# reverb-sys/aeron-cluster-client-cpp

Measured on AMD Instinct MI355X. Metric: SBE records encoded+decoded/sec (device-resident), 256 B Order msgs, higher is better.
Workload: dtype u8; 1 GPU; roundtrip_fixed256_orders; records_per_gpu=1000000, record_bytes=256, encode=wire-correct TopicMessage, packed SoA input, decode=parse_message descriptors (views) + sequence_number evaluation, parallelism=shard1, input_sets=3

## Files before the change

### aeron-cluster-client-cpp_amd/csrc/sbe_codec.hip

```cpp
#include <hip/hip_ext.h>
#include <hip/hip_runtime.h>
#include <dlfcn.h>
#include <rccl/rccl.h>

#include <chrono>
#include <mutex>
#include <new>
#include <thread>
#include <type_traits>

#include <cstdint>
#include <cstdio>
#include <cstring>

#include "../../include/sbecodec.h"

namespace {

constexpr int kWave = 64;
constexpr int kTile = 64;
#ifndef SBE_DEC_WIN
#define SBE_DEC_WIN 16384
#endif
#ifndef SBE_DEC_WIN_WIDE
#define SBE_DEC_WIN_WIDE 20480
#endif
constexpr uint32_t kWin = SBE_DEC_WIN;
constexpr uint32_t kWinWide = SBE_DEC_WIN_WIDE;
constexpr uint64_t kWideAvg = 256;
#ifndef SBE_DEC_SMALL_AVG
#define SBE_DEC_SMALL_AVG 112
#endif
#ifndef SBE_DEC_MID_AVG
#define SBE_DEC_MID_AVG 204
#endif
#ifndef SBE_DEC_WIN_MID
#define SBE_DEC_WIN_MID 15360
#endif
constexpr uint32_t kWinMid = SBE_DEC_WIN_MID, kWinSmall = 8192;
#ifndef SBE_DEC_WIN_LARGE
#define SBE_DEC_WIN_LARGE 13312
#endif
#ifndef SBE_DEC_LARGE_AVG
#define SBE_DEC_LARGE_AVG 320
#endif
constexpr uint32_t kWinLarge = SBE_DEC_WIN_LARGE;
constexpr uint64_t kLargeAvg = SBE_DEC_LARGE_AVG;
constexpr uint64_t kMidAvg = SBE_DEC_MID_AVG, kSmallAvg = SBE_DEC_SMALL_AVG;

__device__ __forceinline__ uint32_t swz(uint32_t i) { return i ^ ((i >> 6) & 28u); }

__device__ __forceinline__ uint4 lds_read_chunk(const uint32_t* win, uint32_t c) {
    const uint32_t x = (c >> 4) & 31u;
    return *reinterpret_cast<const uint4*>(win + ((4u * c) ^ (x & 28u)));
}

__device__ __forceinline__ void lds_write_chunk(uint32_t* win, uint32_t c, uint4 v) {
    const uint32_t x = (c >> 4) & 31u;
    *reinterpret_cast<uint4*>(win + ((4u * c) ^ (x & 28u))) = v;
}

__device__ __forceinline__ uint32_t lds_dw(const uint32_t* win, uint32_t i) { return win[swz(i)]; }
__device__ __forceinline__ uint4 lds_read_chunk_raw(const uint32_t* win, uint32_t c) {
    return *reinterpret_cast<const uint4*>(win + ((4u * c) ^ (((c >> 4) & 31u) & 28u)));
}

template <int kCtrl, int kRowMask = 0xf>
__device__ __forceinline__ uint32_t dpp0(uint32_t v) {
    return (uint32_t)__builtin_amdgcn_update_dpp(0, (int)v, kCtrl, kRowMask, 0xf, false);
}

__device__ __forceinline__ uint32_t wave_incl_scan(uint32_t v, int lane) {
    (void)lane;
    v += dpp0<0x111>(v);
    v += dpp0<0x112>(v);
    v += dpp0<0x114>(v);
    v += dpp0<0x118>(v);
    v += dpp0<0x142, 0xa>(v);
    v += dpp0<0x143, 0xc>(v);
    return v;
}

__device__ __forceinline__ uint32_t ceil_div_small(uint32_t a, uint32_t b) {
    const uint32_t x = a + b - 1;
    uint32_t q = (uint32_t)((float)x * __builtin_amdgcn_rcpf((float)b));
    q += (q + 1) * b <= x;
    q -= q * b > x;
    return q;
}

__device__ __forceinline__ uint32_t wave_incl_max(uint32_t v) {
    v = max(v, dpp0<0x111>(v));
    v = max(v, dpp0<0x112>(v));
    v = max(v, dpp0<0x114>(v));
    v = max(v, dpp0<0x118>(v));
    v = max(v, dpp0<0x142, 0xa>(v));
    v = max(v, dpp0<0x143, 0xc>(v));
    return v;
}

template <int kCtrl, int kRowMask = 0xf>
__device__ __forceinline__ uint64_t dpp_add64(uint64_t v) {
    const uint32_t lo = (uint32_t)v, hi = (uint32_t)(v >> 32);
    const uint32_t tlo = dpp0<kCtrl, kRowMask>(lo), thi = dpp0<kCtrl, kRowMask>(hi);
    const uint32_t nlo = lo + tlo;
    return ((uint64_t)(hi + thi + (nlo < lo ? 1u : 0u)) << 32) | nlo;
}
__device__ __forceinline__ uint64_t wave_incl_scan64(uint64_t v, int lane) {
    (void)lane;
    v = dpp_add64<0x111>(v);
    v = dpp_add64<0x112>(v);
    v = dpp_add64<0x114>(v);
    v = dpp_add64<0x118>(v);
    v = dpp_add64<0x142, 0xa>(v);
    v = dpp_add64<0x143, 0xc>(v);
    return v;
}

__device__ __forceinline__ uint32_t lane_u32(uint32_t v, int l) { return __builtin_amdgcn_readlane(v, l); }
__device__ __forceinline__ uint64_t lane_u64(uint64_t v, int l) {
    const uint32_t hi = (uint32_t)__builtin_amdgcn_readlane((uint32_t)(v >> 32), l);
    const uint32_t lo = (uint32_t)__builtin_amdgcn_readlane((uint32_t)v, l);
    return ((uint64_t)hi << 32) | lo;
}

__device__ __forceinline__ uint64_t wave_sum64(uint64_t v) { return lane_u64(wave_incl_scan64(v, 0), kWave - 1); }

__device__ __forceinline__ uint64_t uniform64(uint64_t v) {
    uint32_t lo = __builtin_amdgcn_readfirstlane((uint32_t)v);
    uint32_t hi = __builtin_amdgcn_readfirstlane((uint32_t)(v >> 32));
    return ((uint64_t)hi << 32) | lo;
}

__device__ __forceinline__ uint32_t byte_mask_bits(uint32_t nbytes) {
    return nbytes >= 4 ? 0xffffffffu : ((1u << (8u * nbytes)) - 1u);
}

typedef unsigned int u32x4 __attribute__((ext_vector_type(4)));
typedef __attribute__((address_space(1))) const uint32_t g_u32;
typedef __attribute__((address_space(1))) const u32x4 g_u32x4;
__device__ __forceinline__ uint32_t gload32(uintptr_t addr) { return *reinterpret_cast<g_u32*>(addr); }
__device__ __forceinline__ uint4 gload128(uintptr_t addr) {
    const u32x4 v = *reinterpret_cast<g_u32x4*>(addr);
    return make_uint4(v.x, v.y, v.z, v.w);
}
__device__ __forceinline__ uint4 gload128_nt(uintptr_t addr) {
    const u32x4 v = __builtin_nontemporal_load(reinterpret_cast<g_u32x4*>(addr));
    return make_uint4(v.x, v.y, v.z, v.w);
}
template <typename T>
__device__ __forceinline__ void dst_store(T* p, T v) {
    __builtin_nontemporal_store(v, p);
}

constexpr int kSbThreads = 1024;
constexpr int kTilesPerSb = 2 * kWave;
constexpr int kSbRecMin = kTilesPerSb * 32;

template <int kPre_, int kBlk_, int kNF_, bool kTM_, int kRpt_>
struct Lay {
    static constexpr int kRpt = kRpt_;
    static constexpr int kLpr = kWave / kRpt;
    static constexpr int kSbRec = kTilesPerSb * kRpt;
    static_assert((kRpt == 32 || kRpt == 64) && kSbRec % kSbThreads == 0 && kSbThreads % kRpt == 0, "tile shape");
    static constexpr int32_t kPre = kPre_;
    static constexpr int32_t kBlk = kBlk_;
    static constexpr int kNF = kNF_;
    static constexpr bool kTM = kTM_;
    static constexpr int32_t kLit = kPre + 8 + kBlk;
    static constexpr int32_t kS0 = kLit + 2;
    static constexpr int32_t kOvh = kLit + 2 * kNF;
    static constexpr int32_t ovh(bool trunc) { return kOvh - (trunc ? 8 : 0); }
    static constexpr int kStoreRows0 = kNF == 2 ? (kRpt == 64 ? 5 : 3) : 8;
};
#ifndef SBE_TM_RPT
#define SBE_TM_RPT 32
#endif
#ifndef SBE_TMS_RPT
#define SBE_TMS_RPT 32
#endif
#ifndef SBE_L3_RPT
#define SBE_L3_RPT 64
#endif
using LayTM = Lay<0, 16, 5, true, SBE_TM_RPT>;
using LayTMS = Lay<32, 16, 5, true, SBE_TMS_RPT>;
using LayL2 = Lay<0, 12, 2, false, 64>;
using LayL3 = Lay<0, 12, 3, false, SBE_L3_RPT>;
static_assert(LayTM::kOvh == SBE_TM_WIRE_OVERHEAD && LayTM::ovh(true) == SBE_TM_REF_OVERHEAD, "TM layout");
static_assert(LayL2::kOvh == SBE_LITE_OVERHEAD(2) && LayTMS::kPre == SBE_SESSION_HDR_LEN, "layouts");
#define SBE_TILE_SHAPE(LY)                                                  \
    [[maybe_unused]] constexpr int kRpt = LY::kRpt, kLpr = LY::kLpr; \
    [[maybe_unused]] constexpr int kSbRec = LY::kSbRec

struct EncArgs {
    const uint8_t* arena;
    const uint32_t* str_off;
    const uint32_t* str_len;
    const uint64_t* timestamp;
    const uint32_t* topic_id;
    uint32_t tmpl;
    int64_t term_id, sess_id;
    uint64_t n;
    uint64_t ts_default;
    uint8_t* out;
    uint64_t cap;
    uint64_t* out_off;
    uint8_t* status;
    uint64_t* tsum;
    uint64_t* bsum;
    uint8_t* sink;
};
constexpr int kSinkBytes = 16 * 64;

constexpr int kOutAux = 2;
constexpr int kOutAuxKeep = 0;
constexpr uint64_t kKeepMin = 96ull << 20, kKeepMax = 256ull << 20;

enum : int { kLenWire = 0, kLenRef = 1, kLenPub = 2 };

template <class LY, int kLen>
__device__ __forceinline__ void rec_sizes(const EncArgs& a, uint64_t r, uint32_t& out_b, uint64_t& in_b,
                                          uint8_t& st) {
    uint32_t sum = 0;
    uint64_t sum_in = 0;
    st = SBE_ENC_OK;
    if (r < a.n) {
#pragma unroll
        for (int f = LY::kNF - 1; f >= 0; --f) {
            const uint32_t L = a.str_len[LY::kNF * r + f];
            sum += kLen == kLenPub ? (L & 0xffffu) : L;
            sum_in += L;
            if (kLen != kLenPub && L > SBE_VAR_MAX_LEN) st = (uint8_t)(SBE_ENC_E109_TOPIC + f);
        }
    }
    const uint32_t ovh = (uint32_t)LY::ovh(kLen == kLenRef);
    out_b = (r < a.n && st == SBE_ENC_OK) ? ovh + sum : 0u;
    in_b = r < a.n ? sum_in : 0u;
}


template <class LY, bool kPacked, int kLen>
__global__ __launch_bounds__(kSbThreads) void sbe_enc_sums(EncArgs a) {
    SBE_TILE_SHAPE(LY);
    __shared__ uint64_t tl[2][kTilesPerSb];
    const int tid = threadIdx.x;
    const uint64_t sb = blockIdx.x;
#pragma unroll
    for (int j = 0; j < kSbRec / kSbThreads; ++j) {
        const uint64_t r = sb * kSbRec + (uint64_t)j * kSbThreads + tid;
        uint32_t ob;
        uint64_t ib;
        uint8_t st;
        rec_sizes<LY, kLen>(a, r, ob, ib, st);
        const int lane = tid & (kWave - 1);
        const uint32_t so = wave_incl_scan(ob, lane);
        const uint32_t o31 = lane_u32(so, 31), o63 = lane_u32(so, kWave - 1);
        uint64_t i31 = 0, i63 = 0;
        if (kPacked) {
            const uint64_t si = wave_incl_scan64(ib, lane);
            i31 = lane_u64(si, 31);
            i63 = lane_u64(si, kWave - 1);
        }
        if (lane == 0) {
            const int tile = j * (kSbThreads / kRpt) + (kWave / kRpt) * (tid / kWave);
            if (kRpt == 32) {
                tl[0][tile] = o31;
                tl[1][tile] = i31;
                tl[0][tile + 1] = o63 - o31;
                tl[1][tile + 1] = i63 - i31;
            } else {
                tl[0][tile] = o63;
                tl[1][tile] = i63;
            }
        }
    }
    __syncthreads();
    if (tid < kWave) {
        const int lane = tid;
        constexpr int kPer = kTilesPerSb / kWave;
        const uint64_t o0 = tl[0][kPer * lane], o1 = kPer == 2 ? tl[0][kPer * lane + 1] : 0ull;
        const uint64_t i0 = tl[1][kPer * lane], i1 = kPer == 2 ? tl[1][kPer * lane + 1] : 0ull;
        const uint64_t io = wave_incl_scan64(o0 + o1, lane), ii = wave_incl_scan64(i0 + i1, lane);
        const uint64_t eo = io - o0 - o1, ei = ii - i0 - i1;
        const uint64_t t0 = sb * kTilesPerSb + kPer * lane;
        *reinterpret_cast<ulonglong2*>(a.tsum + 2 * t0) = make_ulonglong2(eo, ei);
        if (kPer == 2) *reinterpret_cast<ulonglong2*>(a.tsum + 2 * t0 + 2) = make_ulonglong2(eo + o0, ei + i0);
        if (lane == kWave - 1) *reinterpret_cast<ulonglong2*>(a.bsum + 2 * sb) = make_ulonglong2(io, ii);
    }
}

#ifndef SBE_PACK_MIN_WAVES
#define SBE_PACK_MIN_WAVES 1
#endif
#ifndef SBE_ENC_WIN
#define SBE_ENC_WIN 8192
#endif
constexpr int32_t kEW = SBE_ENC_WIN;
constexpr int32_t kEWIn = SBE_ENC_WIN + 256;

constexpr int32_t kInSlack = 64;
constexpr int32_t kRowPad = 16;
constexpr int32_t kWoutBytes = kEW + (kEW / 256) * kRowPad;
constexpr int32_t kWinBytes = kEWIn + 2 * kInSlack;

typedef __attribute__((address_space(3))) uint8_t lds_u8;
typedef __attribute__((address_space(3))) const uint8_t lds_cu8;
typedef __attribute__((address_space(3))) uint32_t lds_u32;
typedef __attribute__((address_space(3))) const uint32_t lds_cu32;
typedef unsigned int u32x2 __attribute__((ext_vector_type(2)));
typedef __attribute__((address_space(3))) u32x4 lds_u32x4;
typedef __attribute__((address_space(3))) u32x2 lds_u32x2;
__device__ __forceinline__ void lds_store16(lds_u8* p, uint4 v) {
    u32x4 x;
    x.x = v.x; x.y = v.y; x.z = v.z; x.w = v.w;
    *reinterpret_cast<lds_u32x4*>(p) = x;
}

__device__ __forceinline__ uint32_t wout_addr(int32_t d) { return (uint32_t)d + (((uint32_t)d >> 8) * kRowPad); }

struct LdsLin {
    lds_cu8* b;
    __device__ __forceinline__ uint32_t dw(int32_t i) const { return reinterpret_cast<lds_cu32*>(b)[i]; }
};
struct GlbClamp {
    uintptr_t base4;
    int32_t imax;
    __device__ __forceinline__ uint32_t dw(int32_t i) const {
        i = i < 0 ? 0 : (i > imax ? imax : i);
        return gload32(base4 + 4u * (uint32_t)i);
    }
};

__device__ __forceinline__ uint64_t low_bytes64(uint64_t v, int32_t n) { return n >= 8 ? v : v & ((1ull << (8 * n)) - 1); }

struct Writer {
    lds_u8* w;
    int32_t lo, pos;
    uint32_t carry;

    __device__ __forceinline__ void put_dw(int32_t d, uint32_t v) const {
        *reinterpret_cast<lds_u32*>(w + wout_addr(d)) = v;
    }
    __device__ __forceinline__ void put_bytes(int32_t d, uint32_t v, int32_t b0, int32_t b1) const {
        lds_u8* p = w + wout_addr(d);
#pragma unroll
        for (int k = 0; k < 4; ++k)
            if (k >= b0 && k < b1) p[k] = (uint8_t)(v >> (8 * k));
    }
    __device__ __forceinline__ void put_first(int32_t d, uint32_t v) const {
        if (d >= lo) put_dw(d, v); else put_bytes(d, v, lo - d, 4);
    }
    __device__ __forceinline__ void lit(uint64_t v, int32_t n) {
        const int32_t t = pos & 3, d = pos & ~3, total = t + n;
        const uint64_t lo64 = (v << (8 * t)) | carry;
        const uint32_t x0 = (uint32_t)lo64, x1 = (uint32_t)(lo64 >> 32);
        const uint32_t x2 = t ? (uint32_t)(v >> (64 - 8 * t)) : 0u;
        if (total >= 4) put_first(d, x0);
        if (total >= 8) put_dw(d + 4, x1);
        carry = total >= 8 ? x2 : (total >= 4 ? x1 : x0);
        pos += n;
    }
    template <typename Src>
    __device__ __forceinline__ void str(const Src& S, int32_t s, int32_t m) {
        const int32_t t = pos & 3, d = pos & ~3, total = t + m;
        const int32_t u = s - t;
        const uint32_t sh = (uint32_t)u & 3u;
        const int32_t i0 = u >> 2;
        const int32_t nd = total >> 2, rem = total & 3;
        uint32_t prev = S.dw(i0);
        const uint32_t nx = S.dw(i0 + 1);
        const uint32_t w0 = (__builtin_amdgcn_alignbyte(nx, prev, sh) & ~byte_mask_bits((uint32_t)t)) | carry;
        pos += m;
        if (nd == 0) {
            carry = w0 & byte_mask_bits((uint32_t)total);
            return;
        }
        put_first(d, w0);
        prev = nx;
        int32_t k = 1;
        const int32_t kg = 4 - ((d >> 2) & 3);
        for (; k < kg && k < nd; ++k) {
            const uint32_t n0 = S.dw(i0 + k + 1);
            put_dw(d + 4 * k, __builtin_amdgcn_alignbyte(n0, prev, sh));
            prev = n0;
        }
        for (; k + 4 <= nd; k += 4) {
            const uint32_t n0 = S.dw(i0 + k + 1), n1 = S.dw(i0 + k + 2), n2 = S.dw(i0 + k + 3), n3 = S.dw(i0 + k + 4);
            u32x2 lo2, hi2;
            lo2.x = __builtin_amdgcn_alignbyte(n0, prev, sh);
            lo2.y = __builtin_amdgcn_alignbyte(n1, n0, sh);
            hi2.x = __builtin_amdgcn_alignbyte(n2, n1, sh);
            hi2.y = __builtin_amdgcn_alignbyte(n3, n2, sh);
            lds_u8* g = w + wout_addr(d + 4 * k);
            reinterpret_cast<lds_u32x2*>(g)[0] = lo2;
            reinterpret_cast<lds_u32x2*>(g)[1] = hi2;
            prev = n3;
        }
        for (; k < nd; ++k) {
            const uint32_t n0 = S.dw(i0 + k + 1);
            put_dw(d + 4 * k, __builtin_amdgcn_alignbyte(n0, prev, sh));
            prev = n0;
        }
        carry = rem ? (__builtin_amdgcn_alignbyte(S.dw(i0 + nd + 1), prev, sh) & byte_mask_bits((uint32_t)rem)) : 0u;
    }
    __device__ __forceinline__ void flush() const {
        const int32_t t = pos & 3;
        if (t) {
            const int32_t d = pos & ~3;
            put_bytes(d, carry, lo > d ? lo - d : 0, t);
        }
    }
};

__device__ __noinline__ Writer str_global(Writer W, uintptr_t sa, int32_t m) {
    const uintptr_t b4 = sa & ~(uintptr_t)3;
    const int32_t sl = (int32_t)(sa - b4);
    W.str(GlbClamp{b4, (sl + m - 1) >> 2}, sl, m);
    return W;
}

__device__ __forceinline__ void wsync() { __builtin_amdgcn_wave_barrier(); }

constexpr int kStageRegs = (kEWIn / 16 + kWave - 1) / kWave;

#ifdef SBE_PACK_PHASES
__device__ uint64_t g_pack_phase[16384 * 8];
struct Ph {
    uint64_t t, acc[8];
    __device__ void start() {
        t = __builtin_amdgcn_s_memtime();
        for (int k = 0; k < 8; ++k) acc[k] = 0;
    }
    __device__ void lap(int k) {
        const uint64_t n = __builtin_amdgcn_s_memtime();
        acc[k] += n - t;
        t = n;
    }
    __device__ void put(int lane) {
        uint64_t v = 0;
        for (int k = 0; k < 8; ++k) v = lane == k ? acc[k] : v;
        if (lane < 8 && blockIdx.x < 16384) g_pack_phase[8 * blockIdx.x + lane] = v;
    }
};
#else
struct Ph {
    __device__ void start() {}
    __device__ void lap(int) {}
    __device__ void put(int) {}
};
#endif

struct TileIn {
    uint32_t L[5];
    uint64_t ts;
    uint32_t tid;
    uint64_t to, ti, po, pi;
    uint32_t pcount;
};

struct TileSt {
    uint32_t rs, rec_out, ps, pe;
    uint32_t pe_rec;
    uint64_t in0;
    uint32_t L[5];
    uint64_t ts;
    uint32_t tid;
    uint64_t T0;
    uint32_t len;
    uint32_t agg_in;
    uintptr_t in_tile;
    uintptr_t gsrc[5];
    bool wrapped;
    uint32_t agg_out;
    uint64_t tot_in;
};

template <class LY, bool kPacked>
__device__ __forceinline__ TileIn tile_load(const EncArgs& a, uint64_t tile, int lane, uint64_t& sb_next) {
    SBE_TILE_SHAPE(LY);
    TileIn x;
    uint64_t r = tile * kRpt + lane / kLpr;
    r = r < a.n ? r : a.n - 1;
#pragma unroll
    for (int f = 0; f < 5; ++f) x.L[f] = f < LY::kNF ? a.str_len[LY::kNF * r + f] : 0u;
    x.ts = a.timestamp[r];
    x.tid = LY::kTM ? 0u : a.topic_id[r];
    x.to = a.tsum[2 * tile];
    x.ti = kPacked ? a.tsum[2 * tile + 1] : 0ull;
    const uint64_t sbt = tile / kTilesPerSb;
    const uint64_t last_sb = (a.n - 1) / kSbRec;
    uint64_t s = sb_next + (uint64_t)lane;
    s = s < last_sb ? s : last_sb;
    x.po = a.bsum[2 * s];
    x.pi = kPacked ? a.bsum[2 * s + 1] : 0ull;
    x.pcount = sbt > sb_next ? (uint32_t)(sbt - sb_next) : 0u;
    sb_next = sbt > sb_next ? sbt : sb_next;
    return x;
}

template <class LY, bool kPacked, int kLen>
__device__ __forceinline__ TileSt tile_prepare_at(const EncArgs& a, const TileIn& x, uint64_t r_first, uint64_t rend,
                                                  int lane, uint64_t base_out, uint64_t base_in);

template <class LY, bool kPacked, int kLen>
__device__ __forceinline__ TileSt tile_prepare(const EncArgs& a, const TileIn& x, uint64_t tile, int lane,
                                               uint64_t& sp_out, uint64_t& sp_in) {
    SBE_TILE_SHAPE(LY);
    sp_out += wave_sum64((uint32_t)lane < x.pcount ? x.po : 0ull);
    if (kPacked) sp_in += wave_sum64((uint32_t)lane < x.pcount ? x.pi : 0ull);
    const uint64_t base_out = uniform64(sp_out + x.to);
    const uint64_t base_in = kPacked ? uniform64(sp_in + x.ti) : 0ull;
    return tile_prepare_at<LY, kPacked, kLen>(a, x, tile * kRpt, a.n, lane, base_out, base_in);
}

template <class LY, bool kPacked, int kLen>
__device__ __forceinline__ TileSt tile_prepare_at(const EncArgs& a, const TileIn& x, uint64_t r_first, uint64_t rend,
                                                  int lane, uint64_t base_out, uint64_t base_in) {
    SBE_TILE_SHAPE(LY);
    TileSt S;
    const int q = lane % kLpr;
    const uint64_t r = r_first + lane / kLpr;
    const bool valid = r < rend;
    uint64_t sum = 0, sum_in = 0;
    uint8_t st = SBE_ENC_OK;
#pragma unroll
    for (int f = 0; f < 5; ++f) {
        const uint32_t Lx = valid ? x.L[f] : 0u;
        S.L[f] = kLen == kLenPub ? (Lx & 0xffffu) : Lx;
        sum += S.L[f];
        sum_in += Lx;
    }
    if (kLen != kLenPub) {
#pragma unroll
        for (int f = LY::kNF - 1; f >= 0; --f)
            if (S.L[f] > SBE_VAR_MAX_LEN) st = (uint8_t)(SBE_ENC_E109_TOPIC + f);
    }
    const uint32_t ovh = (uint32_t)LY::ovh(kLen == kLenRef);
    const uint32_t rec_out = (valid && st == SBE_ENC_OK) ? ovh + (uint32_t)sum : 0u;
    const uint64_t rec_in = (kPacked && valid) ? sum_in : 0ull;
    S.wrapped = kLen == kLenPub && kPacked && __ballot(sum_in != sum) != 0;
    const uint32_t lo_out = q == 0 ? rec_out : 0u;
    const uint32_t inc_out = wave_incl_scan(lo_out, lane);
    const uint32_t agg_out = lane_u32(inc_out, kWave - 1);
    S.rs = kLpr == 2 ? dpp0<0xa0>(inc_out - lo_out) : inc_out - lo_out;
    S.rec_out = rec_out;
    S.agg_out = agg_out;
    S.tot_in = 0;
    if (kPacked) {
        if (__ballot(!(valid && st == SBE_ENC_OK)) == 0 && !S.wrapped) {
            const uint32_t ovh0 = ovh;
            S.in0 = S.rs - ovh0 * (uint32_t)(lane / kLpr);
            const uint64_t agg_in = agg_out - (uint64_t)ovh0 * kRpt;
            S.agg_in = (uint32_t)agg_in;
            S.tot_in = agg_in;
        } else {
            const uint64_t lo_in = q == 0 ? rec_in : 0ull;
            const uint64_t inc_in = wave_incl_scan64(lo_in, lane);
            const uint64_t agg_in = lane_u64(inc_in, kWave - 1);
            S.agg_in = agg_in < 0x7fffffffull ? (uint32_t)agg_in : 0x7fffffffu;
            S.tot_in = agg_in;
            const uint64_t ex = inc_in - lo_in;
            S.in0 = kLpr == 2 ? ((uint64_t)dpp0<0xa0>((uint32_t)(ex >> 32)) << 32) | dpp0<0xa0>((uint32_t)ex) : ex;
        }
    } else {
        S.agg_in = 0;
        S.in0 = 0;
    }
    S.ts = LY::kTM ? ((valid && x.ts) ? x.ts : a.ts_default) : x.ts;
    S.tid = x.tid;
    const uint32_t re = S.rs + rec_out;
    const uint64_t cap_rel64 = a.cap > base_out ? a.cap - base_out : 0ull;
    uint32_t cap_rel = agg_out;
    if (cap_rel64 < (uint64_t)agg_out) {
        const uint64_t over = __ballot(q == 0 && rec_out != 0 && (uint64_t)re > cap_rel64);
        cap_rel = lane_u32(S.rs, __builtin_ctzll(over));
    }
    if (valid && q == 0) {
        if (st == SBE_ENC_OK && (uint64_t)re > cap_rel64) st = SBE_ENC_OVERFLOW;
        a.out_off[r] = base_out + S.rs;
        if (r == a.n - 1) a.out_off[a.n] = base_out + re;
        if (a.status) a.status[r] = st;
    }
    const uint32_t ps = q == 0 ? S.rs : ((S.rs + (uint32_t)q * rec_out / kLpr + 3) & ~3u);
    const uint32_t pe = q == kLpr - 1 ? re : ((S.rs + (uint32_t)(q + 1) * rec_out / kLpr + 3) & ~3u);
    const uint32_t hi_rec = re < cap_rel ? re : cap_rel;
// ... 1737 lines not shown
        }
    }
    if (d.len[0] == 0) {
#pragma unroll
        for (int k = 0; k < 5; ++k) d.off[k] = d.len[k] = 0;
        d.status = SBE_ST_EG_NONE;
        return;
    }
    d.status = SBE_ST_EG_TM;
}

template <typename R_t>
__device__ void dec_lite(const R_t& R, uint32_t len, Desc& d) {
    d.clear();
    if (len < 8) { d.status = SBE_ST_LITE_NOT_LITE; return; }
    const uint32_t h0 = R.u32(0), h1 = R.u32(4);
    const uint32_t blk = h0 & 0xffffu, tmpl = h0 >> 16, schema = h1 & 0xffffu;
    d.set_hdr(R, 0);
    const uint32_t nf = tmpl == SBE_COMMIT_OFFSET_LITE_TEMPLATE_ID ? 2u
                      : (tmpl == SBE_ORDER_REQUEST_LITE_TEMPLATE_ID || tmpl == SBE_ORDER_NOTIFICATION_LITE_TEMPLATE_ID) ? 3u
                                                                                                                   : 0u;
    if (schema != 1 || nf == 0) { d.status = SBE_ST_LITE_NOT_LITE; return; }
    uint32_t pos = 8u + blk;
    if (pos > len || len < 20) { d.status = SBE_ST_LITE_E100; return; }
#pragma unroll
    for (uint32_t f = 0; f < 3; ++f) {
        if (f >= nf) break;
        if (pos + 2 > len) {
#pragma unroll
            for (int k = 0; k < 5; ++k) d.off[k] = d.len[k] = 0;
            d.status = SBE_ST_LITE_E100;
            return;
        }
        const uint32_t L = R.u16(pos);
        pos += 2;
        if (pos + L > len) {
#pragma unroll
            for (int k = 0; k < 5; ++k) d.off[k] = d.len[k] = 0;
            d.status = SBE_ST_LITE_E100;
            return;
        }
        d.off[f] = pos;
        d.len[f] = L;
        pos += L;
    }
    d.status = SBE_ST_LITE;
    d.ts = R.u64(12);
    d.off[4] = R.u32(8);
}

template <uint32_t kW>
constexpr int dec_regs() {
    static_assert(kW % (16 * kWave) == 0, "decode windows are whole 1 KiB staging rows");
    return (int)(kW / 16 / kWave);
}


template <uint32_t kMode, typename R_t>
__device__ __forceinline__ void dec_record(const R_t& R, uint32_t len, Desc& d) {
    if (kMode == SBE_DEC_ON_EGRESS)
        dec_on_egress(R, len, d);
    else if (kMode == SBE_DEC_LITE)
        dec_lite(R, len, d);
    else
        dec_parse_message(R, len, d);
}

template <uint32_t kMode>
__device__ __noinline__ Desc dec_record_glb(const uint8_t* in, uint64_t rs, uint32_t rl) {
    Desc d;
    d.clear();
    dec_record<kMode>(GlbRec{reinterpret_cast<uintptr_t>(in) + rs}, rl, d);
    return d;
}

template <uint32_t kW>
__device__ __forceinline__ void dec_issue(const DecArgs& a, uint64_t wb, uint64_t we, int lane,
                                          uint4 (&I)[dec_regs<kW>()]) {
    const uint32_t nch = (uint32_t)((we - wb) >> 4);
    const uintptr_t src = reinterpret_cast<uintptr_t>(a.in) + wb;
#pragma unroll
    for (int k = 0; k < dec_regs<kW>(); ++k) {
        const uint32_t ch = lane + kWave * k;
        I[k] = ch < nch ? gload128_nt(src + 16ull * ch) : make_uint4(0, 0, 0, 0);
    }
}

template <uint32_t kMode, uint32_t kW>
__device__ __forceinline__ uint32_t dec_commit(uint32_t* win, uint64_t wb, uint64_t we, bool wide, int lane,
                                               const uint4 (&I)[dec_regs<kW>()]) {
    const uint32_t nch = (uint32_t)((we - wb) >> 4);
#pragma unroll
    for (int k = 0; k < dec_regs<kW>(); ++k) {
        const uint32_t ch = lane + kWave * k;
        if (ch < nch) lds_write_chunk(win, ch, I[k]);
    }
    uint32_t sm = 0;
    if (kMode == SBE_DEC_PARSE_MESSAGE && wide) {
        const uint32_t nrow = (nch + kWave - 1) / kWave;
#pragma unroll
        for (int k = 0; k < dec_regs<kW>(); ++k) {
            if ((uint32_t)k < nrow) {
                Suspect S;
                S.add(I[k]);
                sm |= S.any() ? 1u << k : 0u;
            }
        }
    }
    return sm;
}

template <uint32_t kMode, uint32_t kW>
__device__ __forceinline__ uint32_t dec_stage(const DecArgs& a, uint32_t* win, uint64_t wb, uint64_t we, bool wide,
                                              int lane) {
    uint4 I[dec_regs<kW>()];
    dec_issue<kW>(a, wb, we, lane, I);
    return dec_commit<kMode, kW>(win, wb, we, wide, lane, I);
}

template <uint32_t kMode>
__device__ __forceinline__ void dec_window(const uint32_t* win, uint64_t wb, uint64_t we, uint64_t rs, uint64_t rl,
                                           bool wide, uint32_t sm, bool& done, Desc& d, int lane) {
    bool here = false;
    if (!done && rs >= wb && rs + rl <= we) {
        dec_record<kMode>(LdsRec{win, (uint32_t)(rs - wb)}, (uint32_t)rl, d);
        done = true;
        here = true;
    }
    if (kMode == SBE_DEC_PARSE_MESSAGE) {
        const bool pend = here && (d.flags & kFlSeqPending);
        if (!wide) {
            if (pend)
                d.flags = (d.flags & ~kFlSeqPending) | has_seq_key_lane(LdsRec{win, (uint32_t)(rs - wb)}, d.off[3], d.len[3]);
        } else if (__ballot(pend)) {
            uint32_t hit = 0;
            if (__ballot(sm != 0)) {
                uint32_t hpos;
                bool more;
                window_exact(win, sm, (uint32_t)(we - wb), lane, hpos, more);
                const uint32_t p0 = (uint32_t)(rs - wb) + d.off[3], p1 = p0 + d.len[3];
                if (__ballot(more)) {
                    if (pend) hit = has_seq_key_lane(LdsRec{win, (uint32_t)(rs - wb)}, d.off[3], d.len[3]);
                } else {
                    for (uint64_t m = __ballot(hpos != ~0u); m; m &= m - 1) {
                        const uint32_t x = __builtin_amdgcn_readlane(hpos, __builtin_ctzll(m));
                        const uint32_t xa = x & ~kHitEsc;
                        if (x & kHitEsc) hit |= xa >= p0 && xa < p1 ? SBE_FL_SEQ_ESC : 0u;
                        else hit |= x >= p0 && x + 16 <= p1 ? SBE_FL_SEQ_KEY : 0u;
                    }
                }
            }
            if (pend) d.flags = (d.flags & ~kFlSeqPending) | hit;
        }
    }
}

#ifndef SBE_DEC_MINW
#define SBE_DEC_MINW 3
#endif
#ifdef SBE_SERVE_PROF
__device__ uint64_t g_serve_prof[16];
#define SBE_SVP(k, t) tpk[(k) - 5] = __builtin_amdgcn_s_memrealtime()
#else
#define SBE_SVP(k, t) do { } while (0)
#endif
template <uint32_t kMode, uint32_t kWin>
__device__ __forceinline__ void dec_rest(const DecArgs& a, uint32_t* win, uint64_t T0, uint64_t end, uint64_t rs,
                                         uint64_t rl, bool wide, bool& done, Desc& d, int lane,
                                         uint4 (&I)[dec_regs<kWin>()]) {
    for (;;) {
        bool again = false;
        uint64_t wb = 0;
        for (;;) {
            const uint64_t m = __ballot(!done);
            if (m == 0) break;
            const int f = __builtin_ctzll(m);
            const uint64_t rsf = uniform64(__shfl(rs, f, kWave));
            const uint64_t rlf = uniform64(__shfl(rl, f, kWave));
            if ((rsf & 15) + rlf <= kWin && rsf + rlf <= end && rsf >= (T0 & ~15ull)) {
                wb = rsf & ~15ull;
                again = true;
                break;
            }
            if (lane == f) {
                d = dec_record_glb<kMode>(a.in, rs, (uint32_t)rl);
                done = true;
            }
        }
        if (!again) break;
        const uint64_t we = wb + kWin < end ? wb + kWin : end;
        wsync();
        dec_issue<kWin>(a, wb, we, lane, I);
        const uint32_t sm = dec_commit<kMode, kWin>(win, wb, we, wide, lane, I);
        wsync();
        dec_window<kMode>(win, wb, we, rs, rl, wide, sm, done, d, lane);
    }
}

template <uint32_t kMode, bool kServe>
__device__ __forceinline__ void dec_outputs(const DecArgs& a, uint64_t r, bool valid, uint64_t rs, const Desc& d) {
    if (valid) {
        dst_store(a.status + r, (uint8_t)d.status);
        dst_store(a.flags + r, (uint8_t)d.flags);
        dst_store(reinterpret_cast<uint64_t*>(a.hdr + 4 * r),
                  (uint64_t)((uint32_t)d.hdr[0] | ((uint32_t)d.hdr[1] << 16)) |
                      ((uint64_t)((uint32_t)d.hdr[2] | ((uint32_t)d.hdr[3] << 16)) << 32));
        dst_store(a.ts + r, d.ts);
    }
    if (valid) {
        typedef uint32_t u32x4a4 __attribute__((ext_vector_type(4), aligned(4)));
        u32x4a4 o4, l4;
        o4.x = d.off[0]; o4.y = d.off[1]; o4.z = d.off[2]; o4.w = d.off[3];
        l4.x = d.len[0]; l4.y = d.len[1]; l4.z = d.len[2]; l4.w = d.len[3];
        __builtin_nontemporal_store(o4, reinterpret_cast<u32x4a4*>(a.view_off + 5 * r));
        __builtin_nontemporal_store(d.off[4], a.view_off + 5 * r + 4);
        __builtin_nontemporal_store(l4, reinterpret_cast<u32x4a4*>(a.view_len + 5 * r));
        __builtin_nontemporal_store(d.len[4], a.view_len + 5 * r + 4);
    }
    if (kMode == SBE_DEC_PARSE_MESSAGE && a.seq) {
        const bool cand = valid && d.status == SBE_ST_TM && (d.flags & kSeqCand);
        if (__ballot(cand) && cand)
            a.seq[r] = kServe ? json_seq_eval_call_serve(a.in + rs + d.off[3], d.len[3])
                              : json_seq_eval_call(a.in + rs + d.off[3], d.len[3]);
    }
}

template <uint32_t kMode>
__device__ __forceinline__ void dec_oversize(Desc& d) {
    d.status = kMode == SBE_DEC_ON_EGRESS ? SBE_ST_EG_NONE
             : kMode == SBE_DEC_LITE    ? SBE_ST_LITE_E100
                                        : SBE_ST_ERR_TM_E100;
}

template <uint32_t kMode, uint32_t kWin, bool kServe = false>
__device__ __forceinline__ void dec_tile(const DecArgs& a, uint64_t tile, uint32_t* win) {
#ifdef SBE_SERVE_PROF
    const uint64_t tp0 = __builtin_amdgcn_s_memrealtime();
    uint64_t tpk[4] = {tp0, tp0, tp0, tp0};
#endif
    const int lane = threadIdx.x & (kWave - 1);
    const uint64_t t0 = tile * kTile;
    const uint64_t r = t0 + (uint64_t)lane;
    const bool valid = r < a.n;
    const uint64_t last = t0 + kTile < a.n ? t0 + kTile : a.n;
    const uint64_t T0 = uniform64(a.rec_off[t0]);
    const uint64_t end = (uniform64(a.rec_off[last]) + 15) & ~15ull;
    const uint64_t rc = r < a.n ? r : a.n - 1;
    const uint64_t rs = a.rec_off[rc];
    const uint64_t rl = valid ? a.rec_off[rc + 1] - rs : 0;

    Desc d;
    d.clear();
    bool done = !valid;
    if (valid && rl > 0xffffffffull) {
        dec_oversize<kMode>(d);
        done = true;
    }
    uint64_t wb = T0 & ~15ull;
    uint64_t we = wb + kWin < end ? wb + kWin : (end > wb ? end : wb);
    const bool wide = kServe || __ballot(valid && rl > kSeqLaneRec) != 0;
    uint4 I[dec_regs<kWin>()];
    SBE_SVP(5, tp0);
    dec_issue<kWin>(a, wb, we, lane, I);
    uint32_t sm = dec_commit<kMode, kWin>(win, wb, we, wide, lane, I);
    SBE_SVP(6, tp0);
    bool pre = false;
    uint64_t wb2 = 0, we2 = 0;
    {
        const uint64_t m = __ballot(!(done || (rs >= wb && rs + rl <= we)));
        if (m) {
            const int f = __builtin_ctzll(m);
            const uint64_t rsf = uniform64(__shfl(rs, f, kWave));
            const uint64_t rlf = uniform64(__shfl(rl, f, kWave));
            if ((rsf & 15) + rlf <= kWin && rsf + rlf <= end && rsf >= (T0 & ~15ull)) {
                wb2 = rsf & ~15ull;
                we2 = wb2 + kWin < end ? wb2 + kWin : end;
                pre = true;
                dec_issue<kWin>(a, wb2, we2, lane, I);
            }
        }
    }
    wsync();
    dec_window<kMode>(win, wb, we, rs, rl, wide, sm, done, d, lane);
    if (pre) {
        wsync();
        sm = dec_commit<kMode, kWin>(win, wb2, we2, wide, lane, I);
        wsync();
        dec_window<kMode>(win, wb2, we2, rs, rl, wide, sm, done, d, lane);
    }
    if (__ballot(!done)) dec_rest<kMode, kWin>(a, win, T0, end, rs, rl, wide, done, d, lane, I);
    SBE_SVP(7, tp0);
    dec_outputs<kMode, kServe>(a, r, valid, rs, d);
    SBE_SVP(8, tp0);
#ifdef SBE_SERVE_PROF
    if (kServe && lane == 0)
        for (int k = 0; k < 4; ++k) g_serve_prof[5 + k] += tpk[k] - tp0;
#endif
}

#ifndef SBE_DEC_MINW_WIDE
#define SBE_DEC_MINW_WIDE SBE_DEC_MINW
#endif
template <uint32_t kMode, uint32_t kWin>
__global__ __launch_bounds__(kWave, kWin == kWinWide && kWinWide > 16384 ? 2 : ((kWin == kWinWide || kWin == kWinLarge) ? SBE_DEC_MINW_WIDE : SBE_DEC_MINW)) void sbe_decode_kernel(DecArgs a) {
    __shared__ uint32_t win[kWin / 4];
    dec_tile<kMode, kWin>(a, blockIdx.x, win);
}

__device__ __forceinline__ uint64_t counted_n(const uint64_t* n_dev, uint64_t capacity) {
    const uint64_t c = uniform64(*n_dev);
    return c < capacity ? c : capacity;
}

template <uint32_t kMode, uint32_t kWin>
__global__ __launch_bounds__(kWave, kWin == kWinWide && kWinWide > 16384 ? 2 : ((kWin == kWinWide || kWin == kWinLarge) ? SBE_DEC_MINW_WIDE : SBE_DEC_MINW)) void sbe_decode_counted_kernel(DecArgs a, const uint64_t* n_dev) {
    __shared__ uint32_t win[kWin / 4];
    a.n = counted_n(n_dev, a.n);
    if ((uint64_t)blockIdx.x * kTile >= a.n) return;
    dec_tile<kMode, kWin>(a, blockIdx.x, win);
}

thread_local char g_last_error[256] = "";

int record_hip(hipError_t e) {
    if (e == hipSuccess) return SBE_OK;
    std::strncpy(g_last_error, hipGetErrorString(e), sizeof(g_last_error) - 1);
    return SBE_EHIP;
}

constexpr uint64_t kMaxTiles = 0xffffffffull;

uint64_t pack_grid(const void* kernel, uint64_t tiles) {
    struct Entry {
        const void* k;
        int dev;
        uint64_t g;
    };
    static thread_local Entry cache[32] = {};
    int dev = 0;
    if (hipGetDevice(&dev) != hipSuccess) dev = 0;
    uint64_t g = 0;
    for (const Entry& e : cache)
        if (e.k == kernel && e.dev == dev) g = e.g;
    if (g == 0) {
        int per_cu = 0, cus = 0;
        if (hipOccupancyMaxActiveBlocksPerMultiprocessor(&per_cu, kernel, kWave, 0) != hipSuccess || per_cu < 1)
            per_cu = 1;
        if (hipDeviceGetAttribute(&cus, hipDeviceAttributeMultiprocessorCount, dev) != hipSuccess || cus < 1)
            cus = 256;
        g = (uint64_t)per_cu * (uint64_t)cus;
        for (Entry& e : cache)
            if (e.k == nullptr) {
                e = Entry{kernel, dev, g};
                break;
            }
    }
    if (g > (uint64_t)(kWave - 1) * kTilesPerSb) g = (uint64_t)(kWave - 1) * kTilesPerSb;
    return tiles < g ? tiles : g;
}

struct ProfRing {
    static constexpr int kCap = 256;
    hipEvent_t ev[kCap][2];
    int head = 0, count = 0;
    uint64_t launches = 0;
    bool ready = false;
};
thread_local int g_prof_every = 0;
thread_local ProfRing g_prof[2];

hipError_t prof_ready(ProfRing& R) {
    if (!R.ready) {
        for (int i = 0; i < ProfRing::kCap; ++i)
            for (int j = 0; j < 2; ++j) {
                const hipError_t e = hipEventCreate(&R.ev[i][j]);
                if (e != hipSuccess) return e;
            }
        R.ready = true;
    }
    return hipSuccess;
}

void prof_slot(int which, hipEvent_t* start, hipEvent_t* stop) {
    *start = *stop = nullptr;
    if (g_prof_every <= 0) return;
    ProfRing& R = g_prof[which];
    if (R.launches++ % (uint64_t)g_prof_every != 0) return;
    if (!R.ready) return;
    *start = R.ev[R.head][0];
    *stop = R.ev[R.head][1];
}
void prof_commit(int which, hipEvent_t start) {
    if (!start) return;
    ProfRing& R = g_prof[which];
    R.head = (R.head + 1) % ProfRing::kCap;
    if (R.count < ProfRing::kCap) ++R.count;
}


struct FragScan {
    uint32_t dp;
    uint32_t sg;
    int32_t lb;
    int32_t le;
    uint64_t B, E;
};
constexpr uint32_t kFsCount = 0x7fffffffu;
__host__ __device__ __forceinline__ uint32_t fs_dp(const FragScan& e) { return e.dp & kFsCount; }
__host__ __device__ __forceinline__ uint32_t fs_sg(const FragScan& e) { return e.sg & kFsCount; }
struct FragScanOp {
    __host__ __device__ FragScan operator()(const FragScan& a, const FragScan& b) const {
        const bool Aa = (a.sg >> 31) != 0, Ab = (b.sg >> 31) != 0, Ca = (a.dp >> 31) != 0, Cb = (b.dp >> 31) != 0;
        const uint32_t C = (Ca || (Cb && Aa)) ? 0x80000000u : 0u, A = (Aa && Ab) ? 0x80000000u : 0u;
        return FragScan{((fs_dp(a) + fs_dp(b)) & kFsCount) | C, ((fs_sg(a) + fs_sg(b)) & kFsCount) | A,
                        a.lb > b.lb ? a.lb : b.lb, a.le > b.le ? a.le : b.le,
                        (Ab ? a.B : 0ull) + b.B, a.E + (Cb ? a.B : 0ull) + b.E};
    }
};

struct FragArgs {
    const uint8_t* in;
    const uint64_t* frag_off;
    const uint8_t* flags;
    uint64_t n;
    uint8_t* out;
    uint64_t* msg_off;
    uint64_t* counts;
    FragScan* el;
    FragScan* sc;
    uint64_t* msize;
    uint64_t* mfirst;
    uint64_t* mlast;
    uint64_t* big;
};
constexpr uint64_t kFcBig = 64 * 1024, kFcPiece = 64 * 1024;

__device__ __forceinline__ bool frag_single(uint8_t f) {
    return (f & (SBE_FRAG_BEGIN | SBE_FRAG_END)) == (SBE_FRAG_BEGIN | SBE_FRAG_END);
}

#ifndef SBE_FS_PER
#define SBE_FS_PER 4
#endif
constexpr int kFsPer = SBE_FS_PER, kFsThreads = 256, kFsBlk = kFsPer * kFsThreads;
__device__ __forceinline__ FragScan fs_identity() { return FragScan{0u, 0x80000000u, -1, -1, 0ull, 0ull}; }
__device__ __forceinline__ FragScan fs_elem(const FragArgs& a, uint64_t i) {
    if (i >= a.n) return fs_identity();
    const uint8_t f = a.flags[i];
    const bool single = frag_single(f);
    const bool begin = (f & SBE_FRAG_BEGIN) != 0, endf = (f & SBE_FRAG_END) != 0;
    const uint64_t len = a.frag_off[i + 1] - a.frag_off[i];
    FragScan e;
    e.dp = ((single || endf) ? 1u : 0u) | ((!single && endf) ? 0x80000000u : 0u);
    e.sg = (single ? 1u : 0u) | ((single || (!begin && !endf)) ? 0x80000000u : 0u);
    e.lb = (!single && begin) ? (int32_t)i : -1;
    e.le = (!single && endf) ? (int32_t)i : -1;
    e.B = (!single && !endf) ? len : 0ull;
    e.E = (single || endf) ? len : 0ull;
    return e;
}
__device__ __forceinline__ FragScan fs_shfl_up(const FragScan& v, int d) {
    FragScan t;
    t.dp = __shfl_up(v.dp, d, kWave);
    t.sg = __shfl_up(v.sg, d, kWave);
    t.lb = __shfl_up(v.lb, d, kWave);
    t.le = __shfl_up(v.le, d, kWave);
    t.B = __shfl_up(v.B, d, kWave);
    t.E = __shfl_up(v.E, d, kWave);
    return t;
}
__device__ __forceinline__ FragScan fs_wave_scan(FragScan v, int lane) {
#pragma unroll
    for (int d = 1; d < kWave; d <<= 1) {
        const FragScan t = fs_shfl_up(v, d);
        if (lane >= d) v = FragScanOp{}(t, v);
    }
    return v;
}
__device__ __forceinline__ FragScan fs_block(const FragArgs& a, uint64_t b, FragScan (&e)[kFsPer], FragScan* wt,
                                             FragScan& before) {
    const int tid = threadIdx.x, lane = tid & (kWave - 1), w = tid / kWave;
    const uint64_t i0 = b * kFsBlk + (uint64_t)tid * kFsPer;
#pragma unroll
    for (int k = 0; k < kFsPer; ++k) e[k] = fs_elem(a, i0 + k);
#pragma unroll
    for (int k = 1; k < kFsPer; ++k) e[k] = FragScanOp{}(e[k - 1], e[k]);
    const FragScan inc = fs_wave_scan(e[kFsPer - 1], lane);
    const FragScan up = fs_shfl_up(inc, 1);
    const FragScan ex = lane ? up : fs_identity();
    if (lane == kWave - 1) wt[w] = inc;
    __syncthreads();
    FragScan wpre = fs_identity(), tot = fs_identity();
#pragma unroll
    for (int k = 0; k < kFsThreads / kWave; ++k) {
        if (k < w) wpre = FragScanOp{}(wpre, wt[k]);
        tot = FragScanOp{}(tot, wt[k]);
    }
    before = FragScanOp{}(wpre, ex);
    return tot;
}
__device__ __forceinline__ void frag_reduce_body(const FragArgs& a, FragScan* agg) {
    __shared__ FragScan wt[kFsThreads / kWave];
    const uint64_t b = blockIdx.x;
    FragScan e[kFsPer], before;
    const FragScan tot = fs_block(a, b, e, wt, before);
    if (threadIdx.x == 0) agg[b] = tot;
}
__global__ __launch_bounds__(kFsThreads) void frag_reduce(FragArgs a, FragScan* agg) { frag_reduce_body(a, agg); }
constexpr int kFsbThreads = kFsThreads;
__device__ __forceinline__ void frag_scan_blocks_body(FragScan* agg, uint64_t nb, uint64_t* big) {
    __shared__ FragScan wt[kFsbThreads / kWave];
    const int tid = threadIdx.x, lane = tid & (kWave - 1), w = tid / kWave;
    if (big && tid == 0) big[0] = 0;
    FragScan carry = fs_identity();
    for (uint64_t c0 = 0; c0 < nb; c0 += kFsBlk) {
        const uint64_t j0 = c0 + (uint64_t)tid * kFsPer;
        FragScan e[kFsPer];
#pragma unroll
        for (int k = 0; k < kFsPer; ++k) e[k] = j0 + k < nb ? agg[j0 + k] : fs_identity();
        FragScan r[kFsPer];
        r[0] = e[0];
#pragma unroll
        for (int k = 1; k < kFsPer; ++k) r[k] = FragScanOp{}(r[k - 1], e[k]);
        const FragScan inc = fs_wave_scan(r[kFsPer - 1], lane);
        const FragScan up = fs_shfl_up(inc, 1);
        const FragScan ex = lane ? up : fs_identity();
        __syncthreads();
        if (lane == kWave - 1) wt[w] = inc;
        __syncthreads();
        FragScan wpre = fs_identity(), tot = fs_identity();
#pragma unroll
        for (int k = 0; k < kFsbThreads / kWave; ++k) {
            if (k < w) wpre = FragScanOp{}(wpre, wt[k]);
            tot = FragScanOp{}(tot, wt[k]);
        }
        const FragScan P = FragScanOp{}(carry, FragScanOp{}(wpre, ex));
#pragma unroll
        for (int k = 0; k < kFsPer; ++k)
            if (j0 + k < nb) agg[j0 + k] = k ? FragScanOp{}(P, r[k - 1]) : P;
        carry = FragScanOp{}(carry, tot);
    }
}
__global__ __launch_bounds__(kFsbThreads) void frag_scan_blocks(FragScan* agg, uint64_t nb, uint64_t* big) {
    frag_scan_blocks_body(agg, nb, big);
}

__device__ __noinline__ uint32_t frag_singles_before(const FragArgs& a, const FragScan* pre, uint64_t x, uint64_t b) {
    const uint64_t bx = x / kFsBlk, s = bx * kFsBlk;
    const bool fwd = x - s < s + kFsBlk - 1 - x;
    const uint32_t c = fs_sg(fwd ? pre[bx] : pre[bx + 1]);
    const uintptr_t lo = reinterpret_cast<uintptr_t>(a.flags + (fwd ? s : x + 1)),
                    hi = reinterpret_cast<uintptr_t>(a.flags + (fwd ? x : s + kFsBlk - 1));
    uint32_t cnt = 0;
    for (uintptr_t q = lo & ~(uintptr_t)15; q <= hi && lo <= hi; q += 16) {
        const uint4 w4 = gload128(q);
        const uint32_t w0 = w4.x, w1 = w4.y, w2 = w4.z, w3 = w4.w;
#pragma unroll
        for (int t = 0; t < 4; ++t) {
            const uint32_t w = t == 0 ? w0 : t == 1 ? w1 : t == 2 ? w2 : w3;
            const uintptr_t b0 = q + 4 * t;
            uint32_t m = (w >> 1) & w & 0x40404040u;
            if (b0 < lo) m &= lo - b0 >= 4 ? 0u : ~0u << (8 * (lo - b0));
            if (b0 + 3 > hi) m &= b0 > hi ? 0u : byte_mask_bits((uint32_t)(hi - b0 + 1));
            cnt += __builtin_popcount(m);
        }
    }
    (void)b;
    return fwd ? c + cnt : c - cnt;
}

__device__ __forceinline__ void frag_scan_msgs_body(const FragArgs& a, const FragScan* pre) {
    __shared__ FragScan wt[kFsThreads / kWave];
    __shared__ uint32_t sgl[kFsBlk];
    __shared__ uint64_t stg[kFsBlk];
    uint64_t tv[kFsPer][4];
    uint32_t tj[kFsPer];
    const uint64_t b = blockIdx.x;
    FragScan e[kFsPer], before;
    const FragScan tot = fs_block(a, b, e, wt, before);
    const FragScan P = pre[b];
    const FragScan base = FragScanOp{}(P, before);
    const int tid = threadIdx.x;
    const uint64_t blk0 = b * kFsBlk, i0 = blk0 + (uint64_t)tid * kFsPer;
    FragScan v[kFsPer];
#pragma unroll
    for (int k = 0; k < kFsPer; ++k) {
        v[k] = FragScanOp{}(base, e[k]);
        sgl[tid * kFsPer + k] = fs_sg(v[k]);
    }
    __syncthreads();
    auto sg_at = [&](uint64_t x) -> uint32_t {
        return x >= blk0 ? sgl[x - blk0] : frag_singles_before(a, pre, x, b);
    };
    auto group = [&](const FragScan& x, int64_t le_before, uint64_t& s0, bool& gap) {
        int64_t st = (int64_t)x.lb > le_before + 1 ? (int64_t)x.lb : le_before + 1;
        if (st < 0) st = 0;
        s0 = (uint64_t)st;
        const uint32_t sg0 = s0 ? sg_at(s0 - 1) : 0u;
        gap = fs_sg(x) != sg0;
    };
    const uint32_t j0 = fs_dp(P), nj = fs_dp(tot);
#pragma unroll
    for (int k = 0; k < kFsPer; ++k) tj[k] = ~0u;
#pragma unroll
    for (int k = 0; k < kFsPer; ++k) {
        const uint64_t i = i0 + k;
        if (i >= a.n) break;
        const FragScan& x = v[k];
        const FragScan& prev = k ? v[k - 1] : base;
        const uint8_t f = a.flags[i];
        const uint64_t E0 = i ? prev.E : 0ull;
        const bool single = frag_single(f);
        const uint32_t dp = fs_dp(x);
        if ((single || (f & SBE_FRAG_END)) && dp >= 1 && dp <= a.n) {
            const uint64_t j = dp - 1;
            uint64_t first = i, last = i;
            if (!single) {
                uint64_t s0;
// ... 2546 lines not shown
```

Measured before the change: 6.687 billion records/s.

## Vectorize encode size-sum kernel with per-thread record groups and DPP row reductions

The encode prefix-sum kernel now has each thread load the lengths of four consecutive records with 128-bit loads instead of one record per thread with scalar loads. Per-tile sums come from DPP row-group reductions rather than full wave scans. The 64-bit input-byte sum is derived from the output sum unless some lane has an oversized field. Decode kernels also get 4096-byte code alignment. This targets load instruction count and scan overhead in the sizing pass, at the cost of more registers and a separate tail path.

```diff
diff --git a/aeron-cluster-client-cpp_amd/csrc/sbe_codec.hip b/aeron-cluster-client-cpp_amd/csrc/sbe_codec.hip
--- a/aeron-cluster-client-cpp_amd/csrc/sbe_codec.hip
+++ b/aeron-cluster-client-cpp_amd/csrc/sbe_codec.hip
@@ -162,7 +162,7 @@
     static constexpr int kRpt = kRpt_;
     static constexpr int kLpr = kWave / kRpt;
     static constexpr int kSbRec = kTilesPerSb * kRpt;
-    static_assert((kRpt == 32 || kRpt == 64) && kSbRec % kSbThreads == 0 && kSbThreads % kRpt == 0, "tile shape");
+    static_assert(kRpt == 32 || kRpt == 64, "tile shape");
     static constexpr int32_t kPre = kPre_;
     static constexpr int32_t kBlk = kBlk_;
     static constexpr int kNF = kNF_;
@@ -218,69 +218,108 @@
 
 enum : int { kLenWire = 0, kLenRef = 1, kLenPub = 2 };
 
-template <class LY, int kLen>
-__device__ __forceinline__ void rec_sizes(const EncArgs& a, uint64_t r, uint32_t& out_b, uint64_t& in_b,
-                                          uint8_t& st) {
-    uint32_t sum = 0;
-    uint64_t sum_in = 0;
-    st = SBE_ENC_OK;
-    if (r < a.n) {
-#pragma unroll
-        for (int f = LY::kNF - 1; f >= 0; --f) {
-            const uint32_t L = a.str_len[LY::kNF * r + f];
-            sum += kLen == kLenPub ? (L & 0xffffu) : L;
-            sum_in += L;
-            if (kLen != kLenPub && L > SBE_VAR_MAX_LEN) st = (uint8_t)(SBE_ENC_E109_TOPIC + f);
-        }
-    }
-    const uint32_t ovh = (uint32_t)LY::ovh(kLen == kLenRef);
-    out_b = (r < a.n && st == SBE_ENC_OK) ? ovh + sum : 0u;
-    in_b = r < a.n ? sum_in : 0u;
-}
-
+constexpr int kSumRec = 4;
+typedef u32x4 __attribute__((aligned(4))) u32x4_dw;
+typedef __attribute__((address_space(1))) const u32x4_dw g_u32x4_dw;
+
+template <int kN>
+__device__ __forceinline__ uint32_t row_group_sum(uint32_t v) {
+    static_assert(kN == 8 || kN == 16, "a group lies inside a row");
+    v += dpp0<0x111>(v);
+    v += dpp0<0x112>(v);
+    v += dpp0<0x114>(v);
+    if (kN == 16) v += dpp0<0x118>(v);
+    return v;
+}
+template <int kN>
+__device__ __forceinline__ uint64_t row_group_sum64(uint64_t v) {
+    v = dpp_add64<0x111>(v);
+    v = dpp_add64<0x112>(v);
+    v = dpp_add64<0x114>(v);
+    if (kN == 16) v = dpp_add64<0x118>(v);
+    return v;
+}
 
 template <class LY, bool kPacked, int kLen>
 __global__ __launch_bounds__(kSbThreads) void sbe_enc_sums(EncArgs a) {
     SBE_TILE_SHAPE(LY);
-    __shared__ uint64_t tl[2][kTilesPerSb];
+    constexpr int kNF = LY::kNF, kDw = kSumRec * kNF;
+    constexpr int kLpt = kRpt / kSumRec;
+    constexpr int kTripRec = kSumRec * kSbThreads;
+    constexpr int kTrips = kSbRec / kTripRec;
+    static_assert(kDw % 4 == 0 && kSbRec % kTripRec == 0 && kTripRec % kRpt == 0, "lane grouping");
+    constexpr uint32_t ovh = (uint32_t)LY::ovh(kLen == kLenRef);
+    static_assert((uint64_t)kSbRec * (ovh + kNF * 0xffffull) < (1ull << 32), "superblock output in 32 bits");
+    constexpr uint32_t kPlainMax = kLen == kLenPub ? 0xffffu : (uint32_t)SBE_VAR_MAX_LEN;
+    __shared__ uint32_t tlo[kTilesPerSb];
+    __shared__ uint64_t tli[kTilesPerSb];
     const int tid = threadIdx.x;
     const uint64_t sb = blockIdx.x;
-#pragma unroll
-    for (int j = 0; j < kSbRec / kSbThreads; ++j) {
-        const uint64_t r = sb * kSbRec + (uint64_t)j * kSbThreads + tid;
-        uint32_t ob;
-        uint64_t ib;
-        uint8_t st;
-        rec_sizes<LY, kLen>(a, r, ob, ib, st);
-        const int lane = tid & (kWave - 1);
-        const uint32_t so = wave_incl_scan(ob, lane);
-        const uint32_t o31 = lane_u32(so, 31), o63 = lane_u32(so, kWave - 1);
-        uint64_t i31 = 0, i63 = 0;
-        if (kPacked) {
-            const uint64_t si = wave_incl_scan64(ib, lane);
-            i31 = lane_u64(si, 31);
-            i63 = lane_u64(si, kWave - 1);
-        }
-        if (lane == 0) {
-            const int tile = j * (kSbThreads / kRpt) + (kWave / kRpt) * (tid / kWave);
-            if (kRpt == 32) {
-                tl[0][tile] = o31;
-                tl[1][tile] = i31;
-                tl[0][tile + 1] = o63 - o31;
-                tl[1][tile + 1] = i63 - i31;
-            } else {
-                tl[0][tile] = o63;
-                tl[1][tile] = i63;
+    const uint64_t r_sb = sb * kSbRec + (uint64_t)(kSumRec * tid);
+    const bool whole = (sb + 1) * kSbRec <= a.n;
+    uint32_t L[kTrips][kDw];
+    if (whole) {
+#pragma unroll
+        for (int j = 0; j < kTrips; ++j) {
+            const uintptr_t p = reinterpret_cast<uintptr_t>(a.str_len + kNF * (r_sb + (uint64_t)j * kTripRec));
+#pragma unroll
+            for (int c = 0; c < kDw / 4; ++c) {
+                const u32x4 v = *reinterpret_cast<g_u32x4_dw*>(p + 16u * c);
+                L[j][4 * c] = v.x, L[j][4 * c + 1] = v.y, L[j][4 * c + 2] = v.z, L[j][4 * c + 3] = v.w;
             }
+        }
+    } else {
+        const uint64_t nd = kNF * a.n;
+#pragma unroll
+        for (int j = 0; j < kTrips; ++j) {
+#pragma unroll
+            for (int i = 0; i < kDw; ++i) {
+                const uint64_t d = kNF * (r_sb + (uint64_t)j * kTripRec) + i;
+                const uint32_t v = a.str_len[d < nd ? d : nd - 1];
+                L[j][i] = d < nd ? v : 0u;
+            }
+        }
+    }
+#pragma unroll
+    for (int j = 0; j < kTrips; ++j) {
+        const uint64_t r0 = r_sb + (uint64_t)j * kTripRec;
+        uint32_t out4 = 0;
+        bool odd = false;
+#pragma unroll
+        for (int k = 0; k < kSumRec; ++k) {
+            uint32_t s = 0, m = 0;
+#pragma unroll
+            for (int f = 0; f < kNF; ++f) {
+                const uint32_t Lx = L[j][kNF * k + f];
+                s += kLen == kLenPub ? (Lx & 0xffffu) : Lx;
+                m = max(m, Lx);
+            }
+            const bool past = !whole && r0 + k >= a.n;
+            const bool plain = !past && m <= kPlainMax;
+            out4 += (kLen == kLenPub ? !past : plain) ? ovh + s : 0u;
+            odd |= !plain;
+        }
+        const uint32_t to = row_group_sum<kLpt>(out4);
+        uint64_t ti = to - ovh * (uint32_t)kRpt;
+        if (kPacked && __ballot(odd) != 0) {
+            uint64_t in4 = 0;
+#pragma unroll
+            for (int i = 0; i < kDw; ++i) in4 += L[j][i];
+            ti = row_group_sum64<kLpt>(in4);
+        }
+        if (tid % kLpt == kLpt - 1) {
+            const int tile = j * (kTripRec / kRpt) + tid / kLpt;
+            tlo[tile] = to;
+            tli[tile] = kPacked ? ti : 0ull;
         }
     }
     __syncthreads();
     if (tid < kWave) {
         const int lane = tid;
         constexpr int kPer = kTilesPerSb / kWave;
-        const uint64_t o0 = tl[0][kPer * lane], o1 = kPer == 2 ? tl[0][kPer * lane + 1] : 0ull;
-        const uint64_t i0 = tl[1][kPer * lane], i1 = kPer == 2 ? tl[1][kPer * lane + 1] : 0ull;
-        const uint64_t io = wave_incl_scan64(o0 + o1, lane), ii = wave_incl_scan64(i0 + i1, lane);
+        const uint32_t o0 = tlo[kPer * lane], o1 = kPer == 2 ? tlo[kPer * lane + 1] : 0u;
+        const uint64_t i0 = tli[kPer * lane], i1 = kPer == 2 ? tli[kPer * lane + 1] : 0ull;
+        const uint64_t io = wave_incl_scan(o0 + o1, lane), ii = wave_incl_scan64(i0 + i1, lane);
         const uint64_t eo = io - o0 - o1, ei = ii - i0 - i1;
         const uint64_t t0 = sb * kTilesPerSb + kPer * lane;
         *reinterpret_cast<ulonglong2*>(a.tsum + 2 * t0) = make_ulonglong2(eo, ei);
@@ -2624,7 +2663,7 @@
 #define SBE_DEC_MINW_WIDE SBE_DEC_MINW
 #endif
 template <uint32_t kMode, uint32_t kWin>
-__global__ __launch_bounds__(kWave, kWin == kWinWide && kWinWide > 16384 ? 2 : ((kWin == kWinWide || kWin == kWinLarge) ? SBE_DEC_MINW_WIDE : SBE_DEC_MINW)) void sbe_decode_kernel(DecArgs a) {
+__global__ __attribute__((aligned(4096))) __launch_bounds__(kWave, kWin == kWinWide && kWinWide > 16384 ? 2 : ((kWin == kWinWide || kWin == kWinLarge) ? SBE_DEC_MINW_WIDE : SBE_DEC_MINW)) void sbe_decode_kernel(DecArgs a) {
     __shared__ uint32_t win[kWin / 4];
     dec_tile<kMode, kWin>(a, blockIdx.x, win);
 }
@@ -2635,7 +2674,7 @@
 }
 
 template <uint32_t kMode, uint32_t kWin>
-__global__ __launch_bounds__(kWave, kWin == kWinWide && kWinWide > 16384 ? 2 : ((kWin == kWinWide || kWin == kWinLarge) ? SBE_DEC_MINW_WIDE : SBE_DEC_MINW)) void sbe_decode_counted_kernel(DecArgs a, const uint64_t* n_dev) {
+__global__ __attribute__((aligned(4096))) __launch_bounds__(kWave, kWin == kWinWide && kWinWide > 16384 ? 2 : ((kWin == kWinWide || kWin == kWinLarge) ? SBE_DEC_MINW_WIDE : SBE_DEC_MINW)) void sbe_decode_counted_kernel(DecArgs a, const uint64_t* n_dev) {
     __shared__ uint32_t win[kWin / 4];
     a.n = counted_n(n_dev, a.n);
     if ((uint64_t)blockIdx.x * kTile >= a.n) return;
```

New measurement: 6.713 billion records/s, median of 6. About the same (+0.4%).
